# waabox/domain-mcp-server

Hardware: AMD Instinct MI355X
Metric: classes indexed/sec (higher is better)
Workload: dtype n/a (CPU text indexing); 1 GPU; model=synthetic-java-spring-monorepo-2000-classes, global_batch=2000, parallelism=dp1 (one repo per rank), enrichment=none

## Files before the change

### dmcp/app.py

```python
from __future__ import annotations

import logging
import sys
import threading
from typing import Optional

from .config import Config
from .enrich.backend import EnrichmentBackend, create_backend
from .graph.cache import GraphCache
from .index.git import GitClient
from .index.pipeline import Indexer
from .index.projects import ProjectService
from .models.domain import ProjectStatus
from .query.context import ContextService
from .query.dsl import GraphQueryService
from .store.db import Database
from .store.repositories import Repositories
from .utils.runtime import tune_gc

LOG = logging.getLogger(__name__)


class _StderrHandler(logging.StreamHandler):

    def __init__(self) -> None:
        super().__init__(sys.stderr)

    @property
    def stream(self):
        return sys.stderr

    @stream.setter
    def stream(self, _value) -> None:
        pass


def configure_logging(level: str = "INFO", stream=None) -> None:
    root = logging.getLogger()
    if getattr(configure_logging, "_done", False):
        root.setLevel(level.upper())
        return
    h = logging.StreamHandler(stream) if stream is not None else _StderrHandler()
    h.setFormatter(logging.Formatter("%(asctime)s [%(threadName)s] %(levelname)-5s %(name)s - %(message)s",
                                     "%H:%M:%S"))
    root.handlers[:] = [h]
    root.setLevel(level.upper())
    configure_logging._done = True


def open_database(config: Config):
    if config.database_url:
        from .store.pg import PgDatabase
        db = PgDatabase.from_url(config.database_url, config.database_username, config.database_password)
        LOG.info("Store: %s", db.describe())
        return db
    return Database(config.db_path, background_checkpoint=config.db_background_checkpoint)


class App:
    def __init__(self, config: Optional[Config] = None, *, backend: Optional[EnrichmentBackend] = None,
                 load_graphs: bool = True, db: Optional[Database] = None) -> None:
        self.config = config or Config.from_env()
        self.db = db or open_database(self.config)
        self.repos = Repositories(self.db)
        self.cache = GraphCache(self.repos.projects, refresh_s=self.config.graph_refresh_seconds or None)
        self.git = GitClient(self.config.git_clone_base_path, self.config.git_ssh_key_path,
                             self.config.git_timeout_seconds)
        self.backend = backend if backend is not None else create_backend(self.config)
        self.indexer = Indexer(self.repos, self.cache, self.git, self.backend,
                               batch_size=self.config.enrich_batch_size,
                               max_readme_length=self.config.max_readme_length,
                               description_length=self.config.description_length,
                               parser_threads=self.config.parser_threads,
                               require_enrichment=self.config.require_enrichment_for_analyze,
                               max_source_chars=self.config.enrich_max_source_chars,
                               in_memory_sources=self.config.git_in_memory,
                               in_memory_max_bytes=self.config.git_in_memory_max_mb << 20,
                               lease_ttl_s=self.config.project_lease_seconds,
                               stream_enrichment=self.config.enrich_stream,
                               scan_isolation=self.config.scan_isolation,
                               scan_timeout_s=self.config.scan_timeout_seconds)
        self.projects = ProjectService(self.repos, self.cache)
        self.context = ContextService(self.repos, self.cache)
        self.graph_query = GraphQueryService(self.cache)
        self._scheduler = None
        if self.config.recover_stuck_on_start:
            self.recover_stuck_projects()
        if load_graphs:
            self.cache.load_all()
        tune_gc()

    def recover_stuck_projects(self) -> int:
        import time as _time
        n = 0
        now = _time.time()
        for status in (ProjectStatus.ANALYZING, ProjectStatus.SYNCING):
            for p in self.repos.projects.find_by_status(status):
                owner, until = self.repos.projects.lease_of(p.id)
                if owner is not None and until is not None and float(until) >= now:
                    continue
                p.mark_error()
                self.repos.projects.update_status(p)
                n += 1
                LOG.warning("Recovered project %s stuck in %s -> ERROR", p.name, status.value)
        return n

    def start_scheduler(self) -> None:
        if not self.config.sync_enabled or self._scheduler is not None:
            return
        from .index.scheduler import CronScheduler
        self._scheduler = CronScheduler(self.config.sync_cron, self._scheduled_sync)
        self._scheduler.start()

    def _scheduled_sync(self) -> None:
        LOG.info("Starting scheduled project sync")
        r = self.indexer.sync_all_projects()
        LOG.info("Scheduled sync complete. Success: %d, Failed: %d", r.success_count, r.failure_count)

    def close(self) -> None:
        if self._scheduler is not None:
            self._scheduler.stop()
        self.backend.close()
        self.db.close()


_lock = threading.Lock()
```

### dmcp/store/db.py

```python
from __future__ import annotations

import contextlib
import logging
import os
import sqlite3
import threading
import time
from typing import Iterator, List, Tuple

LOG = logging.getLogger(__name__)

MIGRATIONS: List[Tuple[int, str, str]] = [
    (1, "initial_schema", """
CREATE TABLE IF NOT EXISTS projects (
    id               TEXT PRIMARY KEY,
    name             TEXT NOT NULL,
    repository_url   TEXT NOT NULL UNIQUE,
    clone_location   TEXT,
    default_branch   TEXT DEFAULT 'main',
    status           TEXT NOT NULL DEFAULT 'PENDING',
    last_analyzed_at TEXT,
    last_commit_hash TEXT,
    created_at       TEXT NOT NULL DEFAULT (strftime('%Y-%m-%dT%H:%M:%fZ','now')),
    updated_at       TEXT NOT NULL DEFAULT (strftime('%Y-%m-%dT%H:%M:%fZ','now')),
    description      TEXT,
    graph_data       TEXT
);
CREATE INDEX IF NOT EXISTS idx_projects_status ON projects(status);
CREATE INDEX IF NOT EXISTS idx_projects_name ON projects(name);

CREATE TABLE IF NOT EXISTS source_classes (
    id              TEXT PRIMARY KEY,
    project_id      TEXT NOT NULL REFERENCES projects(id) ON DELETE CASCADE,
    full_class_name TEXT NOT NULL,
    simple_name     TEXT NOT NULL,
    package_name    TEXT,
    class_type      TEXT NOT NULL,
    description     TEXT,
    source_file     TEXT,
    created_at      TEXT NOT NULL DEFAULT (strftime('%Y-%m-%dT%H:%M:%fZ','now')),
    commit_hash     TEXT,
    CONSTRAINT uq_source_classes_project_class UNIQUE(project_id, full_class_name)
);
CREATE INDEX IF NOT EXISTS idx_source_classes_full_name ON source_classes(full_class_name);
CREATE INDEX IF NOT EXISTS idx_source_classes_package ON source_classes(package_name);
CREATE INDEX IF NOT EXISTS idx_source_classes_simple_name ON source_classes(simple_name);
CREATE INDEX IF NOT EXISTS idx_source_classes_type ON source_classes(class_type);
CREATE INDEX IF NOT EXISTS idx_source_classes_project_package ON source_classes(project_id, package_name);

CREATE TABLE IF NOT EXISTS source_methods (
    id             TEXT PRIMARY KEY,
    class_id       TEXT NOT NULL REFERENCES source_classes(id) ON DELETE CASCADE,
    method_name    TEXT NOT NULL,
    description    TEXT,
    business_logic TEXT,
    exceptions     TEXT,
    http_method    TEXT,
    http_path      TEXT,
    line_number    INTEGER,
    created_at     TEXT NOT NULL DEFAULT (strftime('%Y-%m-%dT%H:%M:%fZ','now'))
);
CREATE INDEX IF NOT EXISTS idx_source_methods_class ON source_methods(class_id);
CREATE INDEX IF NOT EXISTS idx_source_methods_name ON source_methods(method_name);
CREATE INDEX IF NOT EXISTS idx_source_methods_http_path ON source_methods(http_path);
CREATE INDEX IF NOT EXISTS idx_source_methods_class_name ON source_methods(class_id, method_name);
CREATE INDEX IF NOT EXISTS idx_source_methods_line ON source_methods(line_number)
    WHERE line_number IS NOT NULL;
CREATE INDEX IF NOT EXISTS idx_source_methods_http_endpoints
    ON source_methods(class_id, http_path, http_method)
    WHERE http_method IS NOT NULL AND http_path IS NOT NULL;

CREATE TABLE IF NOT EXISTS method_parameters (
    id         TEXT PRIMARY KEY,
    method_id  TEXT NOT NULL REFERENCES source_methods(id) ON DELETE CASCADE,
    position   INTEGER NOT NULL,
    class_id   TEXT NOT NULL REFERENCES source_classes(id) ON DELETE CASCADE,
    created_at TEXT NOT NULL DEFAULT (strftime('%Y-%m-%dT%H:%M:%fZ','now')),
    CONSTRAINT uq_method_param_position UNIQUE(method_id, position)
);
CREATE INDEX IF NOT EXISTS idx_method_params_method ON method_parameters(method_id);
CREATE INDEX IF NOT EXISTS idx_method_params_class ON method_parameters(class_id);
"""),
    (2, "optimize_query_indexes", """
-- V4 equivalent: covering index for ORDER BY full_class_name per project;
-- SQLite LIKE-prefix uses the plain package index (no text_pattern_ops).
CREATE INDEX IF NOT EXISTS idx_source_classes_project_ordered
    ON source_classes(project_id, full_class_name);
DROP INDEX IF EXISTS idx_source_classes_project;
CREATE TRIGGER IF NOT EXISTS update_projects_updated_at
    AFTER UPDATE ON projects FOR EACH ROW
    WHEN NEW.updated_at = OLD.updated_at
# ... 64 lines not shown
    line_number    INTEGER,
    created_at     TEXT NOT NULL DEFAULT (strftime('%Y-%m-%dT%H:%M:%fZ','now'))
) WITHOUT ROWID;
CREATE TABLE mp_new (
    id         TEXT PRIMARY KEY,
    method_id  TEXT NOT NULL REFERENCES source_methods(id) ON DELETE CASCADE,
    position   INTEGER NOT NULL,
    class_id   TEXT NOT NULL REFERENCES source_classes(id) ON DELETE CASCADE,
    created_at TEXT NOT NULL DEFAULT (strftime('%Y-%m-%dT%H:%M:%fZ','now')),
    CONSTRAINT uq_method_param_position UNIQUE(method_id, position)
) WITHOUT ROWID;
INSERT INTO sc_new (id, project_id, full_class_name, simple_name, package_name, class_type, description,
                    source_file, created_at, commit_hash)
    SELECT id, project_id, full_class_name, simple_name, package_name, class_type, description, source_file,
           created_at, commit_hash FROM source_classes;
INSERT INTO sm_new (id, class_id, method_name, description, business_logic, exceptions, http_method, http_path,
                    line_number, created_at)
    SELECT id, class_id, method_name, description, business_logic, exceptions, http_method, http_path,
           line_number, created_at FROM source_methods;
INSERT INTO mp_new (id, method_id, position, class_id, created_at)
    SELECT id, method_id, position, class_id, created_at FROM method_parameters;
DROP TABLE method_parameters;
DROP TABLE source_methods;
DROP TABLE source_classes;
ALTER TABLE sc_new RENAME TO source_classes;
ALTER TABLE sm_new RENAME TO source_methods;
ALTER TABLE mp_new RENAME TO method_parameters;
CREATE INDEX idx_source_classes_full_name ON source_classes(full_class_name);
CREATE INDEX idx_source_classes_package ON source_classes(package_name);
CREATE INDEX idx_source_classes_project_package ON source_classes(project_id, package_name);
CREATE INDEX idx_source_methods_class_name ON source_methods(class_id, method_name);
CREATE INDEX idx_source_methods_http_endpoints
    ON source_methods(class_id, http_path, http_method)
    WHERE http_method IS NOT NULL AND http_path IS NOT NULL;
CREATE INDEX idx_method_params_class ON method_parameters(class_id);
"""),
    (7, "project_lease_and_graph_version", """
-- Cross-process project lease (analyze / sync / rebuild / resume take it with
-- a conditional UPDATE and heartbeat it; lease_until is epoch seconds) and a
-- graph version bumped by every full project update, which lets the graph
-- cache of another process (the MCP server) notice a re-analysis.
ALTER TABLE projects ADD COLUMN lease_owner TEXT;
ALTER TABLE projects ADD COLUMN lease_until REAL;
ALTER TABLE projects ADD COLUMN graph_version INTEGER NOT NULL DEFAULT 0;
"""),
    (8, "project_leases_table", """
-- The lease moves to its own table (V7's projects.lease_owner / lease_until
-- are no longer written): SQLite rewrites the whole projects row, with its
-- multi-megabyte graph_data JSON, on every UPDATE of any column.
CREATE TABLE project_leases (
    project_id  TEXT PRIMARY KEY REFERENCES projects(id) ON DELETE CASCADE,
    lease_owner TEXT NOT NULL,
    lease_until REAL NOT NULL
) WITHOUT ROWID;
"""),
    (9, "project_graph_table", """
-- The graph JSON moves out of the projects row into its own table (SQLite
-- only; PostgreSQL keeps the reference's projects.graph_data): SQLite
-- rewrites a whole row, overflow pages included, on any UPDATE, so the
-- status write at the start of every analysis rewrote the previous
-- analysis' ~1.3 MB graph (~2 ms of a ~36 ms analysis on the MI355X host).
-- projects.graph_data stays, always NULL.
CREATE TABLE project_graphs (
    project_id TEXT PRIMARY KEY REFERENCES projects(id) ON DELETE CASCADE,
    graph_data TEXT NOT NULL
);
INSERT INTO project_graphs (project_id, graph_data)
    SELECT id, graph_data FROM projects WHERE graph_data IS NOT NULL;
UPDATE projects SET graph_data = NULL WHERE graph_data IS NOT NULL;
"""),
    (10, "class_enrichment_source", """
-- Which backend wrote a class's enrichment (dmcp.enrich.backend source
-- tags): 'synthetic:...' marks placeholder descriptions -- a random-weight
-- local preset, the echo engine, the offline fake -- that Phase 3 and
-- resume-enrichment redo once a real backend (a checkpoint, the API) is
-- configured.  NULL: never enriched, or enriched before this migration.
ALTER TABLE source_classes ADD COLUMN enrichment_source TEXT;
"""),
]

PAGE_SIZE = 16384


class _Checkpointer:

    def __init__(self, path: str) -> None:
        self.path = path
        self.passes = 0
        self._ev = threading.Event()
        self._stop = False
        self._thread: "threading.Thread | None" = None
        self._lock = threading.Lock()

    def notify(self) -> None:
        if self._thread is None:
            with self._lock:
                if self._thread is None and not self._stop:
                    self._thread = threading.Thread(target=self._run, name="dmcp-wal-checkpoint", daemon=True)
                    self._thread.start()
        self._ev.set()

    def _run(self) -> None:
        conn = sqlite3.connect(self.path, isolation_level=None, check_same_thread=False, timeout=30.0)
        try:
            while True:
                self._ev.wait()
                self._ev.clear()
                try:
                    conn.execute("PRAGMA wal_checkpoint(PASSIVE)").fetchall()
                    self.passes += 1
                except sqlite3.Error as e:
                    LOG.debug("background WAL checkpoint skipped: %s", e)
                if self._stop:
                    return
        finally:
            conn.close()

    def close(self) -> None:
        self._stop = True
        t = self._thread
        if t is not None:
            self._ev.set()
            t.join(timeout=60)


class Database:

    graph_table = True

    def __init__(self, path: str = ":memory:", background_checkpoint: bool = True) -> None:
        self.path = path
        self._local = threading.local()
        self._write_lock = threading.RLock()
        self._shared_memory_conn = None
        self.checkpointer = _Checkpointer(path) if background_checkpoint and path != ":memory:" else None
        if path == ":memory:":
            self._shared_memory_conn = self._open()
        else:
            d = os.path.dirname(os.path.abspath(path))
            os.makedirs(d, exist_ok=True)
        self.migrate()

    def _open(self) -> sqlite3.Connection:
        conn = sqlite3.connect(self.path, check_same_thread=False, isolation_level=None,
                               timeout=30.0)
        conn.row_factory = sqlite3.Row
        conn.execute("PRAGMA foreign_keys = ON")
        if self.path != ":memory:":
            conn.execute(f"PRAGMA page_size = {PAGE_SIZE}")
            for attempt in range(200):
                try:
                    conn.execute("PRAGMA journal_mode = WAL")
                    break
                except sqlite3.OperationalError as e:
                    if "locked" not in str(e) or attempt == 199:
                        raise
                    time.sleep(0.05)
            conn.execute("PRAGMA synchronous = NORMAL")
            if self.checkpointer is not None:
                conn.execute("PRAGMA wal_autocheckpoint = 0")
        conn.execute("PRAGMA temp_store = MEMORY")
        conn.execute("PRAGMA cache_size = -65536")
        return conn

    def is_shared_memory(self) -> bool:
        return self._shared_memory_conn is not None

    @property
    def conn(self) -> sqlite3.Connection:
        if self._shared_memory_conn is not None:
            return self._shared_memory_conn
        c = getattr(self._local, "conn", None)
        if c is None:
            c = self._open()
            self._local.conn = c
        return c

    def committed(self) -> None:
        if self.checkpointer is not None:
            self.checkpointer.notify()

    def close(self) -> None:
        if self.checkpointer is not None:
            self.checkpointer.close()
        c = getattr(self._local, "conn", None)
        if c is not None:
            c.close()
            self._local.conn = None
        if self._shared_memory_conn is not None:
            self._shared_memory_conn.close()
            self._shared_memory_conn = None

    @contextlib.contextmanager
    def transaction(self) -> Iterator[sqlite3.Connection]:
        with self._write_lock:
            conn = self.conn
            depth = getattr(self._local, "tx_depth", 0)
            if self._shared_memory_conn is not None:
                depth = getattr(self, "_mem_tx_depth", 0)
            if depth == 0:
                conn.execute("BEGIN IMMEDIATE")
            self._set_depth(depth + 1)
            try:
                yield conn
            except BaseException:
                self._set_depth(depth)
                if depth == 0:
                    conn.execute("ROLLBACK")
                raise
            else:
                self._set_depth(depth)
                if depth == 0:
                    conn.execute("COMMIT")
                    self.committed()

    @contextlib.contextmanager
    def bulk_transaction(self) -> Iterator[sqlite3.Connection]:
        conn = self.conn
        if self._shared_memory_conn is not None or getattr(self._local, "tx_depth", 0):
            with self.transaction() as c:
                yield c
            return
        with self._write_lock:
            conn.execute("PRAGMA foreign_keys = OFF")
            try:
                with self.transaction() as c:
                    yield c
            finally:
                conn.execute("PRAGMA foreign_keys = ON")

    def _set_depth(self, d: int) -> None:
        if self._shared_memory_conn is not None:
            self._mem_tx_depth = d
        else:
            self._local.tx_depth = d

    def execute(self, sql: str, params=()) -> sqlite3.Cursor:
        if self._shared_memory_conn is not None:
            with self._write_lock:
                return self.conn.execute(sql, params)
        return self.conn.execute(sql, params)

    def query(self, sql: str, params=()) -> List[sqlite3.Row]:
        if self._shared_memory_conn is not None:
            with self._write_lock:
                return self.conn.execute(sql, params).fetchall()
        return self.conn.execute(sql, params).fetchall()

    def query_one(self, sql: str, params=()):
        rows = self.query(sql, params)
        return rows[0] if rows else None

    def migrate(self) -> int:
        with self._write_lock:
            conn = self.conn
            conn.execute("CREATE TABLE IF NOT EXISTS schema_version ("
                         "version INTEGER PRIMARY KEY, description TEXT, "
                         "installed_on TEXT DEFAULT (strftime('%Y-%m-%dT%H:%M:%fZ','now')))")
            done = {r[0] for r in conn.execute("SELECT version FROM schema_version")}
            applied = 0
            for version, desc, sql in MIGRATIONS:
                if version in done:
                    continue
                fk_off = "-- foreign_keys: off" in sql
                if fk_off:
# ... 51 lines not shown
```

### native/srcscan/bulkwriter.cpp

```cpp
#include "bulkwriter.hpp"

#include <cstdlib>

#include <chrono>
#include <stdexcept>

#include "sqlite_min.hpp"

namespace dbw {

namespace {

class Reaper {
  public:
    static void give(std::vector<Batch>&& dead) {
        if (dead.empty()) return;
        static Reaper* r = new Reaper();
        {
            std::lock_guard<std::mutex> g(r->mu_);
            r->queue_.push_back(std::move(dead));
        }
        r->cv_.notify_one();
    }

  private:
    Reaper() { std::thread([this] { loop(); }).detach(); }
    void loop() {
        for (;;) {
            std::vector<Batch> dead;
            {
                std::unique_lock<std::mutex> g(mu_);
                cv_.wait(g, [this] { return !queue_.empty(); });
                dead = std::move(queue_.front());
                queue_.pop_front();
            }
        }
    }
    std::mutex mu_;
    std::condition_variable cv_;
    std::deque<std::vector<Batch>> queue_;
};

struct Conn {
    sqlite3* db = nullptr;
    ~Conn() {
        if (db) sqlite3_close_v2(db);
    }
    void exec(const char* sql) {
        char* err = nullptr;
        if (sqlite3_exec(db, sql, nullptr, nullptr, &err) != sqlite_min::OK) {
            std::string m = err ? err : sqlite3_errmsg(db);
            sqlite3_free(err);
            throw std::runtime_error(std::string(sql) + ": " + m);
        }
    }
    int64_t run(const Batch& b) {
        sqlite3_stmt* st = nullptr;
        if (sqlite3_prepare_v2(db, b.sql.c_str(), static_cast<int>(b.sql.size()), &st, nullptr) != sqlite_min::OK)
            throw std::runtime_error("prepare: " + b.sql + ": " + sqlite3_errmsg(db));
        struct Fin {
            sqlite3_stmt* s;
            ~Fin() { sqlite3_finalize(s); }
        } fin{st};
        const int n = b.ncols;
        if (sqlite3_bind_parameter_count(st) != n)
            throw std::runtime_error("parameter count mismatch for: " + b.sql);
        const size_t rows = n ? b.values.size() / n : 1;
        for (size_t r = 0; r < rows; ++r) {
            const Value* v = n ? &b.values[r * n] : nullptr;
            for (int c = 0; c < n; ++c) {
                const Value& x = v[c];
                int rc = sqlite_min::OK;
                switch (x.kind) {
                    case Value::Null: rc = sqlite3_bind_null(st, c + 1); break;
                    case Value::Int: rc = sqlite3_bind_int64(st, c + 1, x.i); break;
                    case Value::Real: rc = sqlite3_bind_double(st, c + 1, x.d); break;
                    case Value::Text:
                        rc = sqlite3_bind_text(st, c + 1, x.p, x.n, sqlite_min::STATIC);
                        break;
                }
                if (rc != sqlite_min::OK) throw std::runtime_error(std::string("bind: ") + sqlite3_errmsg(db));
            }
            int rc = sqlite3_step(st);
            if (rc != sqlite_min::DONE && rc != sqlite_min::ROW)
                throw std::runtime_error("step: " + b.sql + ": " + sqlite3_errmsg(db));
            sqlite3_reset(st);
        }
        return static_cast<int64_t>(rows);
    }
};

}

BulkWriter::BulkWriter(std::string path, int busy_timeout_ms, std::vector<Batch> setup)
    : path_(std::move(path)), busy_ms_(busy_timeout_ms), setup_(std::move(setup)) {
    thread_ = std::thread([this] { run(); });
}

BulkWriter::~BulkWriter() {
    if (joined_) return;
    if (commit_requested_)
        wait();
    else
        abort();
}

void BulkWriter::push(Item it) {
    {
        std::lock_guard<std::mutex> g(mu_);
        queue_.push_back(std::move(it));
    }
    cv_.notify_one();
}

bool BulkWriter::pop(Item& out) {
    std::unique_lock<std::mutex> g(mu_);
    cv_.wait(g, [this] { return !queue_.empty(); });
    out = std::move(queue_.front());
    queue_.pop_front();
    return true;
}

void BulkWriter::put(Batch batch) { push(Item{Op::Rows, std::move(batch)}); }

void BulkWriter::commit() {
    commit_requested_ = true;
    push(Item{Op::Commit, {}});
}

void BulkWriter::abort() {
    {
        std::lock_guard<std::mutex> g(mu_);
        queue_.push_front(Item{Op::Abort, {}});
    }
    cv_.notify_one();
    wait();
}

std::string BulkWriter::wait() {
    if (!joined_) {
        if (thread_.joinable()) thread_.join();
        joined_ = true;
    }
    return error_;
}

void BulkWriter::run() {
    Conn c;
    bool in_tx = false;
    try {
        if (sqlite3_open_v2(path_.c_str(), &c.db, sqlite_min::OPEN_READWRITE | sqlite_min::OPEN_NOMUTEX, nullptr) !=
            sqlite_min::OK)
            throw std::runtime_error("open " + path_ + ": " + (c.db ? sqlite3_errmsg(c.db) : "out of memory"));
        sqlite3_busy_timeout(c.db, busy_ms_);
        c.exec("PRAGMA synchronous = NORMAL");
        c.exec("PRAGMA temp_store = MEMORY");
        c.exec("PRAGMA cache_size = -65536");
        c.exec("PRAGMA foreign_keys = OFF");
        {
            static const long long mmap_bytes = [] {
                const char* e = std::getenv("DMCP_WRITER_MMAP");
                return e ? std::atoll(e) : (1LL << 30);
            }();
            if (mmap_bytes > 0) {
                const std::string q = "PRAGMA mmap_size = " + std::to_string(mmap_bytes);
                c.exec(q.c_str());
            }
        }
        using clock = std::chrono::steady_clock;
        auto ms = [](clock::time_point a, clock::time_point b) {
            return std::chrono::duration<double, std::milli>(b - a).count();
        };
        auto t0 = clock::now();
        open_ms_ = ms(t_start_, t0);
        c.exec("BEGIN IMMEDIATE");
        in_tx = true;
        for (const Batch& b : setup_) c.run(b);
        setup_.clear();
        setup_ms_ = ms(t0, clock::now());
        t_setup_ = clock::now();
        constexpr size_t kReapGroup = 16;
        std::vector<Batch> dead;
        dead.reserve(kReapGroup);
        static const bool reap = [] {
            const char* e = std::getenv("DMCP_WRITER_REAPER");
            return e == nullptr || e[0] != '0';
        }();
        for (;;) {
            Item it;
            auto tw = clock::now();
            pop(it);
            idle_ms_ += ms(tw, clock::now());
            if (it.op == Op::Abort) {
                c.exec("ROLLBACK");
                in_tx = false;
                error_ = "aborted";
                return;
            }
            if (it.op == Op::Commit) {
                auto tc = clock::now();
                c.exec("COMMIT");
                commit_ms_ = ms(tc, clock::now());
                t_commit_ = tc;
                t_end_ = clock::now();
                Reaper::give(std::move(dead));
                in_tx = false;
                return;
            }
            auto tr = clock::now();
            rows_written_ += c.run(it.batch);
            auto tf = clock::now();
            rows_ms_ += ms(tr, tf);
            if (reap) {
                dead.push_back(std::move(it.batch));
                if (dead.size() >= kReapGroup) {
                    Reaper::give(std::move(dead));
                    dead = std::vector<Batch>();
                    dead.reserve(kReapGroup);
                }
            } else
                Batch(std::move(it.batch));
            free_ms_ += ms(tf, clock::now());
        }
    } catch (const std::exception& e) {
        error_ = e.what();
        if (in_tx && c.db) sqlite3_exec(c.db, "ROLLBACK", nullptr, nullptr, nullptr);
    }
}

}
```

### native/srcscan/bulkwriter.hpp

```cpp
#pragma once

#include <condition_variable>
#include <cstdint>
#include <deque>
#include <memory>
#include <mutex>
#include <chrono>
#include <string>
#include <thread>
#include <utility>
#include <vector>

namespace dbw {

struct Value {
    enum Kind : uint8_t { Null, Int, Real, Text } kind = Null;
    int32_t n = 0;
    union {
        int64_t i;
        double d;
        const char* p;
    };
    Value() : i(0) {}
};

struct Batch {
    std::string sql;
    int ncols = 0;
    std::vector<Value> values;
    std::deque<std::string> owned;
    std::shared_ptr<const void> keep;
};

class BulkWriter {
  public:
    BulkWriter(std::string path, int busy_timeout_ms, std::vector<Batch> setup);
    ~BulkWriter();
    BulkWriter(const BulkWriter&) = delete;
    BulkWriter& operator=(const BulkWriter&) = delete;

    void put(Batch batch);
    void commit();
    void abort();
    std::string wait();
    int64_t rows_written() const { return rows_written_; }
    double setup_ms() const { return setup_ms_; }
    double rows_ms() const { return rows_ms_; }
    double commit_ms() const { return commit_ms_; }
    double idle_ms() const { return idle_ms_; }
    double free_ms() const { return free_ms_; }
    double open_ms() const { return open_ms_; }
    static double secs(std::chrono::steady_clock::time_point t) {
        return std::chrono::duration<double>(t.time_since_epoch()).count();
    }
    double t_start() const { return secs(t_start_); }
    double t_setup() const { return secs(t_setup_); }
    double t_commit() const { return secs(t_commit_); }
    double t_end() const { return secs(t_end_); }

  private:
    enum class Op { Rows, Commit, Abort };
    struct Item {
        Op op;
        Batch batch;
    };
    void run();
    void push(Item it);
    bool pop(Item& out);

    std::string path_;
    int busy_ms_;
    std::vector<Batch> setup_;
    std::mutex mu_;
    std::condition_variable cv_;
    std::deque<Item> queue_;
    std::thread thread_;
    std::string error_;
    int64_t rows_written_ = 0;
    double setup_ms_ = 0, rows_ms_ = 0, commit_ms_ = 0, idle_ms_ = 0, open_ms_ = 0, free_ms_ = 0;
    std::chrono::steady_clock::time_point t_start_ = std::chrono::steady_clock::now();
    std::chrono::steady_clock::time_point t_setup_{}, t_commit_{}, t_end_{};
    bool joined_ = false;
    bool commit_requested_ = false;
};

}
```

### native/srcscan/pymodule.cpp

```cpp
#include <pybind11/pybind11.h>
#include <pybind11/stl.h>
#include <sys/random.h>

#include <cctype>
#include <chrono>
#include <cstring>
#include <deque>
#include <memory>
#include <thread>
#include <unordered_map>
#include <vector>

#include "bulkwriter.hpp"
#include "gitobj.hpp"
#include "graphjson.hpp"
#include "srcscan.hpp"
#include "staticrows.hpp"
#include "wire.hpp"

namespace py = pybind11;

namespace {

using staticrows::StaticRowsEmitter;
// ... 876 lines not shown
            std::string commit;
            bool ok;
            {
                py::gil_scoped_release release;
                ok = gitobj::resolve_commit(git_dir, refs, commit);
            }
            if (!ok) return py::none();
            return pystr(commit);
        },
        py::arg("git_dir"), py::arg("refs"),
        "Commit id of the first resolvable ref (tags peeled) from loose refs/objects; None = ask git.");
    m.def(
        "list_tree_loose",
        [](const std::vector<std::string>& object_dirs, const std::string& commit) -> py::object {
            std::vector<std::pair<std::string, std::string>> entries;
            bool ok;
            {
                py::gil_scoped_release release;
                ok = gitobj::list_tree(object_dirs, commit, entries);
            }
            if (!ok) return py::none();
            py::list out(entries.size());
            for (size_t i = 0; i < entries.size(); ++i) {
                PyObject* path = PyUnicode_DecodeUTF8(entries[i].first.data(),
                                                      static_cast<Py_ssize_t>(entries[i].first.size()), "strict");
                if (!path) {
                    PyErr_Clear();
                    return py::none();
                }
                out[i] = py::make_tuple(py::reinterpret_steal<py::str>(path), pystr(entries[i].second));
            }
            return out;
        },
        py::arg("object_dirs"), py::arg("commit"),
        "(path, blob id) of the commit's regular files in ls-tree -r order, or None unless all trees are loose.");

    py::class_<dbw::BulkWriter>(m, "BulkWriter",
                                "One SQLite write transaction on a worker thread (see bulkwriter.hpp).")
        .def(py::init([](const std::string& path, int busy_timeout_ms, py::list setup) {
                 std::vector<dbw::Batch> stmts;
                 for (auto item : setup) {
                     auto tup = item.cast<py::tuple>();
                     stmts.push_back(to_batch(tup[0].cast<std::string>(), tup[1]));
                 }
                 return new dbw::BulkWriter(path, busy_timeout_ms, std::move(stmts));
             }),
             py::arg("path"), py::arg("busy_timeout_ms"), py::arg("setup"))
        .def(
            "put", [](dbw::BulkWriter& w, const std::string& sql, py::handle rows) { w.put(to_batch(sql, rows)); },
            py::arg("sql"), py::arg("rows"))
        .def("commit", &dbw::BulkWriter::commit)
        .def("abort", &dbw::BulkWriter::abort, py::call_guard<py::gil_scoped_release>())
        .def(
            "wait",
            [](dbw::BulkWriter& w) {
                std::string err;
                {
                    py::gil_scoped_release release;
                    err = w.wait();
                }
                if (!err.empty()) throw std::runtime_error("bulk write failed: " + err);
                return w.rows_written();
            })
        .def("phase1_rows", &phase1_rows, py::arg("order"), py::arg("units"), py::arg("ids"), py::arg("pid"),
             py::arg("now"), py::arg("commit_hash"), py::arg("class_sql"), py::arg("method_sql"),
             py::arg("param_sql"), py::arg("method_info_cls"), py::arg("chunk") = 256,
             py::arg("graph_targets") = py::none(), py::arg("pre_ids") = py::none(),
             "Phase 1 rows of the parsed units straight into this writer (see phase1_rows in pymodule.cpp)")
        .def_property_readonly("rows_written", &dbw::BulkWriter::rows_written)
        .def("timings", [](const dbw::BulkWriter& w) {
            py::dict d;
            d["setup_ms"] = w.setup_ms();
            d["rows_ms"] = w.rows_ms();
            d["commit_ms"] = w.commit_ms();
            d["idle_ms"] = w.idle_ms();
            d["free_ms"] = w.free_ms();
            d["open_ms"] = w.open_ms();
            d["t_start_s"] = w.t_start();
            d["t_setup_s"] = w.t_setup();
            d["t_commit_s"] = w.t_commit();
            d["t_end_s"] = w.t_end();
            return d;
        });
    m.attr("ABI_VERSION") = 7;
}
```

### native/srcscan/sqlite_min.hpp

```cpp
#pragma once

#include <cstdint>

extern "C" {
struct sqlite3;
struct sqlite3_stmt;
typedef int64_t sqlite3_int64;

int sqlite3_open_v2(const char* filename, sqlite3** db, int flags, const char* vfs);
int sqlite3_close_v2(sqlite3* db);
int sqlite3_busy_timeout(sqlite3* db, int ms);
int sqlite3_exec(sqlite3* db, const char* sql, int (*cb)(void*, int, char**, char**), void* arg, char** errmsg);
void sqlite3_free(void* p);
int sqlite3_prepare_v2(sqlite3* db, const char* sql, int n, sqlite3_stmt** stmt, const char** tail);
int sqlite3_bind_null(sqlite3_stmt* s, int i);
int sqlite3_bind_int64(sqlite3_stmt* s, int i, sqlite3_int64 v);
int sqlite3_bind_double(sqlite3_stmt* s, int i, double v);
int sqlite3_bind_text(sqlite3_stmt* s, int i, const char* v, int n, void (*destructor)(void*));
int sqlite3_bind_parameter_count(sqlite3_stmt* s);
int sqlite3_step(sqlite3_stmt* s);
int sqlite3_reset(sqlite3_stmt* s);
int sqlite3_finalize(sqlite3_stmt* s);
const char* sqlite3_errmsg(sqlite3* db);
}

namespace sqlite_min {
constexpr int OK = 0;
constexpr int ROW = 100;
constexpr int DONE = 101;
constexpr int OPEN_READWRITE = 0x00000002;
constexpr int OPEN_NOMUTEX = 0x00008000;
inline void (*const STATIC)(void*) = nullptr;
}
```

Baseline: 55200 classes/s.

## Keep persistent writer worker threads with cached SQLite connections per database file

Adds a per-file registry of writer hosts whose worker threads keep an open SQLite connection, applied pragmas and a prepared-statement cache across BulkWriter sessions. New writers reuse an idle worker, so they skip the connection open, pragma setup and statement re-preparation, and repeated setup PRAGMAs are skipped. It is on by default and can be disabled with DMCP_WRITER_HOST=0. The cost is added lifecycle complexity: stale hosts are detected by inode, evicted by LRU, cleared in forked children and closed from App/Database close. Long-lived connections and detached orphan threads are a risk.

```diff
diff --git a/dmcp/app.py b/dmcp/app.py
--- a/dmcp/app.py
+++ b/dmcp/app.py
@@ -14,7 +14,7 @@
 from .models.domain import ProjectStatus
 from .query.context import ContextService
 from .query.dsl import GraphQueryService
-from .store.db import Database
+from .store.db import Database, close_writer_hosts
 from .store.repositories import Repositories
 from .utils.runtime import tune_gc
 
@@ -122,6 +122,9 @@
             self._scheduler.stop()
         self.backend.close()
         self.db.close()
+        path = getattr(self.db, "path", None)
+        if isinstance(path, str):
+            close_writer_hosts(path)
 
 
 _lock = threading.Lock()
diff --git a/dmcp/store/db.py b/dmcp/store/db.py
--- a/dmcp/store/db.py
+++ b/dmcp/store/db.py
@@ -6,7 +6,7 @@
 import sqlite3
 import threading
 import time
-from typing import Iterator, List, Tuple
+from typing import Iterator, List, Optional, Tuple
 
 LOG = logging.getLogger(__name__)
 
@@ -237,6 +237,17 @@
 PAGE_SIZE = 16384
 
 
+def close_writer_hosts(path: Optional[str] = None) -> int:
+    if path == ":memory:":
+        return 0
+    try:
+        from .. import _srcscan
+    except ImportError:
+        return 0
+    fn = getattr(_srcscan, "close_writer_hosts", None)
+    return int(fn(path)) if fn is not None else 0
+
+
 class _Checkpointer:
 
     def __init__(self, path: str) -> None:
@@ -336,6 +347,7 @@
             self.checkpointer.notify()
 
     def close(self) -> None:
+        close_writer_hosts(self.path)
         if self.checkpointer is not None:
             self.checkpointer.close()
         c = getattr(self._local, "conn", None)
diff --git a/native/srcscan/bulkwriter.cpp b/native/srcscan/bulkwriter.cpp
--- a/native/srcscan/bulkwriter.cpp
+++ b/native/srcscan/bulkwriter.cpp
@@ -1,9 +1,14 @@
 #include "bulkwriter.hpp"
+
+#include <pthread.h>
+#include <sys/stat.h>
+#include <sys/types.h>
 
 #include <cstdlib>
 
 #include <chrono>
 #include <stdexcept>
+#include <unordered_map>
 
 #include "sqlite_min.hpp"
 
@@ -41,10 +46,26 @@
     std::deque<std::vector<Batch>> queue_;
 };
 
-struct Conn {
+}
+
+struct WriterConn {
     sqlite3* db = nullptr;
-    ~Conn() {
+    bool keep = false;
+    std::unordered_map<std::string, sqlite3_stmt*> stmts;
+    std::vector<std::string> pragmas;
+    static constexpr size_t kMaxStmts = 64;
+
+    WriterConn() = default;
+    WriterConn(const WriterConn&) = delete;
+    WriterConn& operator=(const WriterConn&) = delete;
+    ~WriterConn() { close(); }
+
+    void close() {
+        for (auto& kv : stmts) sqlite3_finalize(kv.second);
+        stmts.clear();
+        pragmas.clear();
         if (db) sqlite3_close_v2(db);
+        db = nullptr;
     }
     void exec(const char* sql) {
         char* err = nullptr;
@@ -54,14 +75,65 @@
             throw std::runtime_error(std::string(sql) + ": " + m);
         }
     }
+    void open(const std::string& path) {
+        if (sqlite3_open_v2(path.c_str(), &db, sqlite_min::OPEN_READWRITE | sqlite_min::OPEN_NOMUTEX, nullptr) !=
+            sqlite_min::OK) {
+            const std::string m = db ? sqlite3_errmsg(db) : "out of memory";
+            close();
+            throw std::runtime_error("open " + path + ": " + m);
+        }
+        try {
+            exec("PRAGMA synchronous = NORMAL");
+            exec("PRAGMA temp_store = MEMORY");
+            exec("PRAGMA cache_size = -65536");
+            exec("PRAGMA foreign_keys = OFF");
+            static const long long mmap_bytes = [] {
+                const char* e = std::getenv("DMCP_WRITER_MMAP");
+                return e ? std::atoll(e) : (1LL << 30);
+            }();
+            if (mmap_bytes > 0) {
+                const std::string q = "PRAGMA mmap_size = " + std::to_string(mmap_bytes);
+                exec(q.c_str());
+            }
+        } catch (...) {
+            close();
+            throw;
+        }
+    }
     int64_t run(const Batch& b) {
         sqlite3_stmt* st = nullptr;
-        if (sqlite3_prepare_v2(db, b.sql.c_str(), static_cast<int>(b.sql.size()), &st, nullptr) != sqlite_min::OK)
-            throw std::runtime_error("prepare: " + b.sql + ": " + sqlite3_errmsg(db));
+        bool cached = false;
+        if (keep) {
+            auto it = stmts.find(b.sql);
+            if (it != stmts.end()) {
+                st = it->second;
+                cached = true;
+            }
+        }
+        if (!st) {
+            if (sqlite3_prepare_v2(db, b.sql.c_str(), static_cast<int>(b.sql.size()), &st, nullptr) != sqlite_min::OK)
+                throw std::runtime_error("prepare: " + b.sql + ": " + sqlite3_errmsg(db));
+            if (keep && st) {
+                if (stmts.size() >= kMaxStmts) {
+                    for (auto& kv : stmts) sqlite3_finalize(kv.second);
+                    stmts.clear();
+                }
+                stmts.emplace(b.sql, st);
+                cached = true;
+            }
+        }
         struct Fin {
             sqlite3_stmt* s;
-            ~Fin() { sqlite3_finalize(s); }
-        } fin{st};
+            bool cached;
+            ~Fin() {
+                if (!cached)
+                    sqlite3_finalize(s);
+                else {
+                    sqlite3_reset(s);
+                    sqlite3_clear_bindings(s);
+                }
+            }
+        } fin{st, cached};
         const int n = b.ncols;
         if (sqlite3_bind_parameter_count(st) != n)
             throw std::runtime_error("parameter count mismatch for: " + b.sql);
@@ -88,13 +160,284 @@
         }
         return static_cast<int64_t>(rows);
     }
+    bool pragma_applied(const std::string& sql) const {
+        for (const std::string& p : pragmas)
+            if (p == sql) return true;
+        return false;
+    }
 };
 
+
+struct WriterHost {
+    std::string real;
+    std::string given;
+    dev_t dev = 0;
+    ino_t ino = 0;
+    std::mutex mu;
+    bool closing = false;
+    std::vector<WriterWorker*> idle;
+    std::vector<std::unique_ptr<WriterWorker>> all;
+    uint64_t last_use = 0;
+
+    WriterWorker* take();
+    void close();
+};
+
+class WriterWorker {
+  public:
+    explicit WriterWorker(std::shared_ptr<WriterHost> host) : host_(std::move(host)) {
+        conn.keep = true;
+        thread_ = std::thread([this] { loop(); });
+    }
+    void assign(BulkWriter* job) {
+        {
+            std::lock_guard<std::mutex> g(mu_);
+            job_ = job;
+        }
+        cv_.notify_one();
+    }
+    void ensure_open() {
+        if (!conn.db) conn.open(host_->real);
+    }
+    WriterConn conn;
+
+  private:
+    friend struct WriterHost;
+    void loop() {
+        for (;;) {
+            BulkWriter* job = nullptr;
+            {
+                std::unique_lock<std::mutex> g(mu_);
+                cv_.wait(g, [this] { return job_ != nullptr || stop_; });
+                if (!job_) break;
+                job = job_;
+            }
+            try {
+                ensure_open();
+                job->run(conn);
+                if (!job->error_.empty() && job->error_ != "aborted") conn.close();
+            } catch (const std::exception& e) {
+                job->error_ = e.what();
+                conn.close();
+            }
+            std::shared_ptr<BulkWriter::Done> done = job->done_;
+            bool back = false;
+            {
+                std::lock_guard<std::mutex> h(host_->mu);
+                std::lock_guard<std::mutex> g(mu_);
+                job_ = nullptr;
+                if (!host_->closing) {
+                    host_->idle.push_back(this);
+                    back = true;
+                }
+            }
+            if (!back) {
+                conn.close();
+                done->signal();
+                break;
+            }
+            done->signal();
+        }
+        conn.close();
+        if (orphan_) delete this;
+    }
+
+    std::shared_ptr<WriterHost> host_;
+    std::thread thread_;
+    std::mutex mu_;
+    std::condition_variable cv_;
+    BulkWriter* job_ = nullptr;
+    bool stop_ = false;
+    bool orphan_ = false;
+};
+
+namespace {
+
+struct Registry {
+    std::mutex mu;
+    std::vector<std::shared_ptr<WriterHost>> hosts;
+    uint64_t tick = 0;
+};
+
+constexpr size_t kMaxHosts = 8;
+
+std::atomic<Registry*> g_registry{nullptr};
+
+void forget_hosts_in_child() { g_registry.store(nullptr); }
+
+Registry& registry() {
+    Registry* r = g_registry.load(std::memory_order_acquire);
+    if (r) return *r;
+    static std::once_flag once;
+    std::call_once(once, [] { pthread_atfork(nullptr, nullptr, forget_hosts_in_child); });
+    Registry* fresh = new Registry();
+    if (g_registry.compare_exchange_strong(r, fresh)) return *fresh;
+    delete fresh;
+    return *r;
+}
+
+std::string real_path(const std::string& path) {
+    char* rp = ::realpath(path.c_str(), nullptr);
+    if (!rp) return std::string();
+    std::string out(rp);
+    std::free(rp);
+    return out;
+}
+
+std::shared_ptr<WriterHost> host_for(const std::string& path) {
+    struct stat st;
+    if (::stat(path.c_str(), &st) != 0) return nullptr;
+    const std::string real = real_path(path);
+    if (real.empty()) return nullptr;
+    Registry& reg = registry();
+    std::shared_ptr<WriterHost> found;
+    std::vector<std::shared_ptr<WriterHost>> dead;
+    {
+        std::lock_guard<std::mutex> g(reg.mu);
+        for (size_t i = 0; i < reg.hosts.size();) {
+            auto& h = reg.hosts[i];
+            if (h->real == real && h->dev == st.st_dev && h->ino == st.st_ino) {
+                found = h;
+                ++i;
+            } else if (h->real == real) {
+                dead.push_back(h);
+                reg.hosts.erase(reg.hosts.begin() + i);
+            } else
+                ++i;
+        }
+        if (!found) {
+            found = std::make_shared<WriterHost>();
+            found->real = real;
+            found->given = path;
+            found->dev = st.st_dev;
+            found->ino = st.st_ino;
+            reg.hosts.push_back(found);
+            while (reg.hosts.size() > kMaxHosts) {
+                size_t lru = 0;
+                for (size_t i = 1; i + 1 < reg.hosts.size(); ++i)
+                    if (reg.hosts[i]->last_use < reg.hosts[lru]->last_use) lru = i;
+                dead.push_back(reg.hosts[lru]);
+                reg.hosts.erase(reg.hosts.begin() + lru);
+            }
+        }
+        found->last_use = ++reg.tick;
+    }
+    for (auto& h : dead) h->close();
+    return found;
+}
+
+}
+
+WriterWorker* WriterHost::take() {
+    std::lock_guard<std::mutex> g(mu);
+    if (closing) return nullptr;
+    if (!idle.empty()) {
+        WriterWorker* w = idle.back();
+        idle.pop_back();
+        return w;
+    }
+    return nullptr;
+}
+
+void WriterHost::close() {
+    std::vector<std::unique_ptr<WriterWorker>> stop;
+    {
+        std::lock_guard<std::mutex> g(mu);
+        if (closing) return;
+        closing = true;
+        for (auto& w : all) {
+            bool is_idle = false;
+            for (WriterWorker* i : idle)
+                if (i == w.get()) is_idle = true;
+            if (is_idle)
+                stop.push_back(std::move(w));
+            else {
+                w->orphan_ = true;
+                w->thread_.detach();
+                w.release();
+            }
+        }
+        all.clear();
+        idle.clear();
+    }
+    for (auto& w : stop) {
+        {
+            std::lock_guard<std::mutex> g(w->mu_);
+            w->stop_ = true;
+        }
+        w->cv_.notify_one();
+    }
+    for (auto& w : stop) w->thread_.join();
+}
+
+namespace {
+
+WriterWorker* acquire_worker(const std::string& path) {
+    for (int attempt = 0; attempt < 4; ++attempt) {
+        std::shared_ptr<WriterHost> h = host_for(path);
+        if (!h) return nullptr;
+        if (WriterWorker* w = h->take()) return w;
+        std::lock_guard<std::mutex> g(h->mu);
+        if (h->closing) continue;
+        h->all.emplace_back(new WriterWorker(h));
+        return h->all.back().get();
+    }
+    return nullptr;
+}
+
+}
+
+bool writer_host_enabled() {
+    const char* e = std::getenv("DMCP_WRITER_HOST");
+    return e == nullptr || e[0] != '0';
+}
+
+size_t writer_hosts() {
+    Registry& reg = registry();
+    std::lock_guard<std::mutex> g(reg.mu);
+    return reg.hosts.size();
+}
+
+size_t close_writer_hosts(const std::string* path) {
+    Registry& reg = registry();
+    std::vector<std::shared_ptr<WriterHost>> dead;
+    {
+        const std::string real = path ? real_path(*path) : std::string();
+        std::lock_guard<std::mutex> g(reg.mu);
+        for (size_t i = 0; i < reg.hosts.size();) {
+            auto& h = reg.hosts[i];
+            if (!path || h->given == *path || (!real.empty() && h->real == real)) {
+                dead.push_back(h);
+                reg.hosts.erase(reg.hosts.begin() + i);
+            } else
+                ++i;
+        }
+    }
+    for (auto& h : dead) h->close();
+    return dead.size();
+}
+
+
+void BulkWriter::Done::signal() {
+    std::lock_guard<std::mutex> g(mu);
+    done = true;
+    cv.notify_all();
+}
+
+void BulkWriter::Done::wait() {
+    std::unique_lock<std::mutex> g(mu);
+    cv.wait(g, [this] { return done; });
 }
 
 BulkWriter::BulkWriter(std::string path, int busy_timeout_ms, std::vector<Batch> setup)
     : path_(std::move(path)), busy_ms_(busy_timeout_ms), setup_(std::move(setup)) {
-    thread_ = std::thread([this] { run(); });
+    if (writer_host_enabled()) {
+        if (WriterWorker* w = acquire_worker(path_)) {
+            w->assign(this);
+            return;
+        }
+    }
+    thread_ = std::thread([this] { run_fresh(); });
 }
 
 BulkWriter::~BulkWriter() {
@@ -139,34 +482,30 @@
 
 std::string BulkWriter::wait() {
     if (!joined_) {
+        done_->wait();
         if (thread_.joinable()) thread_.join();
         joined_ = true;
     }
     return error_;
 }
 
-void BulkWriter::run() {
-    Conn c;
+void BulkWriter::run_fresh() {
+    {
+        WriterConn c;
+        try {
+            c.open(path_);
+            run(c);
+        } catch (const std::exception& e) {
+            error_ = e.what();
+        }
+    }
+    done_->signal();
+}
+
+void BulkWriter::run(WriterConn& c) {
     bool in_tx = false;
     try {
-        if (sqlite3_open_v2(path_.c_str(), &c.db, sqlite_min::OPEN_READWRITE | sqlite_min::OPEN_NOMUTEX, nullptr) !=
-            sqlite_min::OK)
-            throw std::runtime_error("open " + path_ + ": " + (c.db ? sqlite3_errmsg(c.db) : "out of memory"));
         sqlite3_busy_timeout(c.db, busy_ms_);
-        c.exec("PRAGMA synchronous = NORMAL");
-        c.exec("PRAGMA temp_store = MEMORY");
-        c.exec("PRAGMA cache_size = -65536");
-        c.exec("PRAGMA foreign_keys = OFF");
-        {
-            static const long long mmap_bytes = [] {
-                const char* e = std::getenv("DMCP_WRITER_MMAP");
-                return e ? std::atoll(e) : (1LL << 30);
-            }();
-            if (mmap_bytes > 0) {
-                const std::string q = "PRAGMA mmap_size = " + std::to_string(mmap_bytes);
-                c.exec(q.c_str());
-            }
-        }
         using clock = std::chrono::steady_clock;
         auto ms = [](clock::time_point a, clock::time_point b) {
             return std::chrono::duration<double, std::milli>(b - a).count();
@@ -175,7 +514,12 @@
         open_ms_ = ms(t_start_, t0);
         c.exec("BEGIN IMMEDIATE");
         in_tx = true;
-        for (const Batch& b : setup_) c.run(b);
+        for (const Batch& b : setup_) {
+            const bool pragma = c.keep && b.sql.compare(0, 7, "PRAGMA ") == 0;
+            if (pragma && c.pragma_applied(b.sql)) continue;
+            c.run(b);
+            if (pragma) c.pragmas.push_back(b.sql);
+        }
         setup_.clear();
         setup_ms_ = ms(t0, clock::now());
         t_setup_ = clock::now();
diff --git a/native/srcscan/bulkwriter.hpp b/native/srcscan/bulkwriter.hpp
--- a/native/srcscan/bulkwriter.hpp
+++ b/native/srcscan/bulkwriter.hpp
@@ -1,5 +1,6 @@
 #pragma once
 
+#include <atomic>
 #include <condition_variable>
 #include <cstdint>
 #include <deque>
@@ -32,6 +33,13 @@
     std::shared_ptr<const void> keep;
 };
 
+struct WriterConn;
+class WriterWorker;
+struct WriterHost;
+
+bool writer_host_enabled();
+size_t writer_hosts();
+size_t close_writer_hosts(const std::string* path);
 class BulkWriter {
   public:
     BulkWriter(std::string path, int busy_timeout_ms, std::vector<Batch> setup);
@@ -64,7 +72,16 @@
         Op op;
         Batch batch;
     };
-    void run();
+    friend class WriterWorker;
+    struct Done {
+        std::mutex mu;
+        std::condition_variable cv;
+        bool done = false;
+        void signal();
+        void wait();
+    };
+    void run(WriterConn& c);
+    void run_fresh();
     void push(Item it);
     bool pop(Item& out);
 
@@ -75,13 +92,14 @@
     std::condition_variable cv_;
     std::deque<Item> queue_;
     std::thread thread_;
+    std::shared_ptr<Done> done_ = std::make_shared<Done>();
     std::string error_;
     int64_t rows_written_ = 0;
     double setup_ms_ = 0, rows_ms_ = 0, commit_ms_ = 0, idle_ms_ = 0, open_ms_ = 0, free_ms_ = 0;
     std::chrono::steady_clock::time_point t_start_ = std::chrono::steady_clock::now();
     std::chrono::steady_clock::time_point t_setup_{}, t_commit_{}, t_end_{};
     bool joined_ = false;
-    bool commit_requested_ = false;
+    std::atomic<bool> commit_requested_{false};
 };
 
 }
diff --git a/native/srcscan/pymodule.cpp b/native/srcscan/pymodule.cpp
--- a/native/srcscan/pymodule.cpp
+++ b/native/srcscan/pymodule.cpp
@@ -982,5 +982,18 @@
             d["t_end_s"] = w.t_end();
             return d;
         });
-    m.attr("ABI_VERSION") = 7;
-}
+    m.def("writer_host_enabled", &dbw::writer_host_enabled,
+          "BulkWriter sessions run on a kept connection per database file (DMCP_WRITER_HOST, default on).");
+    m.def("writer_hosts", &dbw::writer_hosts, "Number of live writer hosts in this process.");
+    m.def(
+        "close_writer_hosts",
+        [](py::object path) {
+            const bool all = path.is_none();
+            const std::string p = all ? std::string() : py::str(path).cast<std::string>();
+            py::gil_scoped_release release;
+            return dbw::close_writer_hosts(all ? nullptr : &p);
+        },
+        py::arg("path") = py::none(),
+        "Closes the writer hosts of the database file `path` (all of them when None); returns how many.");
+    m.attr("ABI_VERSION") = 8;
+}
diff --git a/native/srcscan/sqlite_min.hpp b/native/srcscan/sqlite_min.hpp
--- a/native/srcscan/sqlite_min.hpp
+++ b/native/srcscan/sqlite_min.hpp
@@ -20,6 +20,7 @@
 int sqlite3_bind_parameter_count(sqlite3_stmt* s);
 int sqlite3_step(sqlite3_stmt* s);
 int sqlite3_reset(sqlite3_stmt* s);
+int sqlite3_clear_bindings(sqlite3_stmt* s);
 int sqlite3_finalize(sqlite3_stmt* s);
 const char* sqlite3_errmsg(sqlite3* db);
 }
diff --git a/native/srcscan/writer_host_check.cpp b/native/srcscan/writer_host_check.cpp
--- /dev/null
+++ b/native/srcscan/writer_host_check.cpp
@@ -0,0 +1,282 @@
+#include <sys/stat.h>
+#include <unistd.h>
+
+#include <cstdio>
+#include <cstdlib>
+#include <fstream>
+#include <sstream>
+#include <string>
+#include <thread>
+#include <vector>
+
+#include "bulkwriter.hpp"
+#include "sqlite_min.hpp"
+
+namespace {
+
+constexpr int OPEN_CREATE = 0x00000004;
+
+const char* kClassSql =
+    "INSERT INTO source_classes (id, project_id, full_class_name, simple_name, package_name, class_type, "
+    "description, source_file, created_at, commit_hash) VALUES (?,?,?,?,?,?,?,?,?,?)";
+const char* kMethodSql =
+    "INSERT INTO source_methods (id, class_id, method_name, description, business_logic, exceptions, http_method, "
+    "http_path, line_number, created_at) VALUES (?,?,?,?,?,?,?,?,?,?)";
+const char* kParamSql = "INSERT INTO method_parameters (id, method_id, position, class_id, created_at) VALUES (?,?,?,?,?)";
+const char* kDeletes[] = {
+    "DELETE FROM method_parameters WHERE class_id IN (SELECT id FROM source_classes WHERE project_id = ?)",
+    "DELETE FROM source_methods WHERE class_id IN (SELECT id FROM source_classes WHERE project_id = ?)",
+    "DELETE FROM source_classes WHERE project_id = ?"};
+
+int failures = 0;
+void check(bool ok, const std::string& what) {
+    if (!ok) {
+        std::fprintf(stderr, "FAILED: %s\n", what.c_str());
+        ++failures;
+    }
+}
+
+struct Db {
+    sqlite3* db = nullptr;
+    Db(const std::string& path, int flags) {
+        if (sqlite3_open_v2(path.c_str(), &db, flags, nullptr) != sqlite_min::OK) {
+            std::fprintf(stderr, "cannot open %s\n", path.c_str());
+            std::exit(2);
+        }
+    }
+    ~Db() { sqlite3_close_v2(db); }
+    void exec(const std::string& sql) {
+        if (sqlite3_exec(db, sql.c_str(), nullptr, nullptr, nullptr) != sqlite_min::OK) {
+            std::fprintf(stderr, "%s: %s\n", sql.c_str(), sqlite3_errmsg(db));
+            std::exit(2);
+        }
+    }
+    long long scalar(const std::string& sql) {
+        long long v = -1;
+        auto cb = [](void* out, int, char** cols, char**) {
+            *static_cast<long long*>(out) = cols[0] ? std::atoll(cols[0]) : 0;
+            return 0;
+        };
+        if (sqlite3_exec(db, sql.c_str(), cb, &v, nullptr) != sqlite_min::OK) {
+            std::fprintf(stderr, "%s: %s\n", sql.c_str(), sqlite3_errmsg(db));
+            std::exit(2);
+        }
+        return v;
+    }
+};
+
+void create_database(const std::string& path, const std::string& ddl) {
+    Db db(path, sqlite_min::OPEN_READWRITE | OPEN_CREATE);
+    db.exec("PRAGMA page_size = 16384");
+    db.exec("PRAGMA journal_mode = WAL");
+    db.exec(ddl);
+}
+
+dbw::Value text(dbw::Batch& b, std::string s) {
+    b.owned.push_back(std::move(s));
+    dbw::Value v;
+    v.kind = dbw::Value::Text;
+    v.p = b.owned.back().data();
+    v.n = static_cast<int32_t>(b.owned.back().size());
+    return v;
+}
+
+dbw::Value integer(int64_t i) {
+    dbw::Value v;
+    v.kind = dbw::Value::Int;
+    v.i = i;
+    return v;
+}
+
+std::vector<dbw::Batch> deletes(const std::string& pid) {
+    std::vector<dbw::Batch> out;
+    out.reserve(4);
+    out.emplace_back();
+    out.back().sql = "PRAGMA wal_autocheckpoint = 0";
+    for (const char* sql : kDeletes) {
+        dbw::Batch b;
+        b.sql = sql;
+        b.ncols = 1;
+        b.values.push_back(text(b, pid));
+        out.push_back(std::move(b));
+    }
+    return out;
+}
+
+void put_rows(dbw::BulkWriter& w, const std::string& pid, int n, int gen, long long& rows) {
+    const std::string now = "2024-01-01T00:00:00.000Z";
+    for (int first = 0; first < n; first += 256) {
+        dbw::Batch cls, meth, par;
+        cls.sql = kClassSql;
+        cls.ncols = 10;
+        meth.sql = kMethodSql;
+        meth.ncols = 10;
+        par.sql = kParamSql;
+        par.ncols = 5;
+        for (int k = first; k < n && k < first + 256; ++k) {
+            const std::string cid = pid + "-g" + std::to_string(gen) + "-c" + std::to_string(k);
+            const std::string name = "C" + std::to_string(k);
+            const std::string pkg = "co.check.p" + std::to_string(k % 7);
+            dbw::Value row[] = {text(cls, cid), text(cls, pid), text(cls, pkg + "." + name), text(cls, name),
+                                text(cls, pkg), text(cls, k % 3 ? "CLASS" : "CONTROLLER"), dbw::Value(),
+                                text(cls, "src/main/java/" + name + ".java"), text(cls, now), text(cls, "cafe")};
+            cls.values.insert(cls.values.end(), row, row + 10);
+            for (int j = 0; j < k % 5; ++j) {
+                const std::string mid = cid + "-m" + std::to_string(j);
+                dbw::Value m[] = {text(meth, mid), text(meth, cid), text(meth, "m" + std::to_string(j)), dbw::Value(),
+                                  dbw::Value(), dbw::Value(), k % 3 ? dbw::Value() : text(meth, "GET"),
+                                  k % 3 ? dbw::Value() : text(meth, "/c" + std::to_string(k)), integer(10 + j),
+                                  text(meth, now)};
+                meth.values.insert(meth.values.end(), m, m + 10);
+                dbw::Value p[] = {text(par, mid + "-p0"), text(par, mid), integer(0), text(par, cid), text(par, now)};
+                par.values.insert(par.values.end(), p, p + 5);
+            }
+        }
+        rows += static_cast<long long>(cls.values.size() / 10 + meth.values.size() / 10 + par.values.size() / 5);
+        w.put(std::move(cls));
+        if (!meth.values.empty()) w.put(std::move(meth));
+        if (!par.values.empty()) w.put(std::move(par));
+    }
+}
+
+long long methods_of(int n) {
+    long long m = 0;
+    for (int k = 0; k < n; ++k) m += k % 5;
+    return m;
+}
+
+Db* g_service = nullptr;
+
+void check_rows(const std::string& path, const std::string& pid, int n, int gen, const std::string& what) {
+    Db db(path, sqlite_min::OPEN_READWRITE);
+    const std::string like = pid + "-g" + std::to_string(gen) + "-%";
+    check(db.scalar("SELECT COUNT(*) FROM source_classes WHERE project_id = '" + pid + "'") == n, what + ": classes");
+    check(db.scalar("SELECT COUNT(*) FROM source_classes WHERE project_id = '" + pid + "' AND id LIKE '" + like +
+                    "'") == n, what + ": classes of this generation");
+    check(db.scalar("SELECT COUNT(*) FROM source_methods WHERE class_id LIKE '" + pid + "-g%'") == methods_of(n),
+          what + ": methods");
+    check(db.scalar("SELECT COUNT(*) FROM method_parameters WHERE class_id LIKE '" + like + "'") == methods_of(n),
+          what + ": parameters");
+}
+
+void swap(const std::string& path, const std::string& pid, int n, int gen, char how, const char* label) {
+    dbw::BulkWriter w(path, 5000, deletes(pid));
+    long long rows = 0;
+    put_rows(w, pid, n, gen, rows);
+    if (how == 'e') {
+        dbw::Batch bad;
+        bad.sql = "INSERT INTO no_such_table VALUES (1)";
+        w.put(std::move(bad));
+    }
+    std::string err;
+    if (how == 'a') {
+        w.abort();
+        err = w.wait();
+        check(err == "aborted", std::string(label) + ": abort reported");
+    } else {
+        w.commit();
+        err = w.wait();
+        if (how == 'e')
+            check(err.find("no_such_table") != std::string::npos, std::string(label) + ": the error is reported");
+        else {
+            check(err.empty(), std::string(label) + ": committed (" + err + ")");
+            check(w.rows_written() == rows, std::string(label) + ": rows_written");
+        }
+    }
+    if (g_service) g_service->exec("PRAGMA wal_checkpoint(PASSIVE)");
+    std::printf("  %-28s open %6.2f  setup %6.2f  rows %6.2f  commit %5.2f ms  %s\n", label, w.open_ms(), w.setup_ms(),
+                w.rows_ms(), w.commit_ms(), err.c_str());
+}
+
+void sequences(const std::string& dir, const std::string& ddl, int n, bool host) {
+    setenv("DMCP_WRITER_HOST", host ? "1" : "0", 1);
+    std::printf("DMCP_WRITER_HOST=%d\n", host ? 1 : 0);
+    const std::string path = dir + (host ? "/host.db" : "/fresh.db");
+    create_database(path, ddl);
+    g_service = new Db(path, sqlite_min::OPEN_READWRITE);
+    g_service->exec("PRAGMA wal_autocheckpoint = 0");
+    swap(path, "p1", n, 1, 'c', "swap 1 (empty tables)");
+    swap(path, "p1", n, 2, 'c', "swap 2");
+    check_rows(path, "p1", n, 2, "swap 2");
+    swap(path, "p1", n, 3, 'a', "swap 3 (aborted)");
+    check_rows(path, "p1", n, 2, "after the abort");
+    swap(path, "p1", n, 4, 'c', "swap 4");
+    check_rows(path, "p1", n, 4, "swap 4");
+    swap(path, "p1", n, 5, 'e', "swap 5 (failing batch)");
+    check_rows(path, "p1", n, 4, "after the failed swap");
+    swap(path, "p1", n, 6, 'c', "swap 6");
+    check_rows(path, "p1", n, 6, "swap 6");
+    check(dbw::writer_hosts() == (host ? 1u : 0u), "one host for one file");
+
+    {
+        dbw::BulkWriter a(path, 5000, deletes("p1"));
+        std::thread other([&] { swap(path, "p2", n / 2 + 1, 1, 'c', "overlapping swap (p2)"); });
+        long long rows = 0;
+        put_rows(a, "p1", n, 7, rows);
+        a.commit();
+        check(a.wait().empty(), "overlapping swap (p1) committed");
+        other.join();
+    }
+    check_rows(path, "p1", n, 7, "overlapping p1");
+    check_rows(path, "p2", n / 2 + 1, 1, "overlapping p2");
+    check(dbw::writer_hosts() == (host ? 1u : 0u), "still one host");
+
+    check(dbw::close_writer_hosts(&path) == (host ? 1u : 0u), "close by path");
+    check(dbw::writer_hosts() == 0, "no host after the close");
+    swap(path, "p1", n, 8, 'c', "swap 8 (new host)");
+    delete g_service;
+    g_service = nullptr;
+    unlink(path.c_str());
+    unlink((path + "-wal").c_str());
+    unlink((path + "-shm").c_str());
+    create_database(path, ddl);
+    swap(path, "p1", 3, 1, 'c', "swap on the replaced file");
+    check_rows(path, "p1", 3, 1, "replaced file");
+    check(dbw::writer_hosts() == (host ? 1u : 0u), "the old file's host is gone");
+
+    {
+        dbw::BulkWriter w(path, 5000, deletes("p1"));
+        long long rows = 0;
+        put_rows(w, "p1", 5, 2, rows);
+        dbw::close_writer_hosts(nullptr);
+        check(dbw::writer_hosts() == 0, "no host after close-all");
+        w.commit();
+        check(w.wait().empty(), "the open session committed after the close");
+        check(w.rows_written() == rows, "rows of the open session");
+    }
+    check_rows(path, "p1", 5, 2, "after close with a session open");
+    check(dbw::writer_hosts() == 0, "the closed host does not come back");
+    swap(path, "p1", 4, 3, 'c', "swap after close-all");
+    check_rows(path, "p1", 4, 3, "after close-all");
+    {
+        dbw::BulkWriter w(dir + "/missing.db", 5000, {});
+        w.commit();
+        check(w.wait().find("open ") == 0, "a missing file is an open error");
+    }
+    dbw::close_writer_hosts(nullptr);
+    for (const char* suffix : {"", "-wal", "-shm"}) unlink((path + suffix).c_str());
+}
+
+}
+
+int main(int argc, char** argv) {
+    if (argc < 2) {
+        std::fprintf(stderr, "usage: writer_host_check DDL_FILE [classes=600]\n");
+        return 2;
+    }
+    std::ifstream in(argv[1]);
+    std::stringstream ddl;
+    ddl << in.rdbuf();
+    if (!in || ddl.str().empty()) {
+        std::fprintf(stderr, "cannot read %s\n", argv[1]);
+        return 2;
+    }
+    const int n = argc > 2 ? std::atoi(argv[2]) : 600;
+    char dir[] = "/tmp/writer_host_check_XXXXXX";
+    if (!mkdtemp(dir)) return 2;
+    sequences(dir, ddl.str(), n, true);
+    sequences(dir, ddl.str(), n, false);
+    rmdir(dir);
+    std::printf("%s: %d classes per swap\n", failures ? "FAILED" : "ok", n);
+    return failures ? 1 : 0;
+}
```

Result: slower. 47900 classes/s (-13.2%).
